# Iheckzza/FeatureMatching

Hardware: AMD Instinct MI355X
Metric: image-pairs/sec at 640x480 (coarse corr + dual-softmax mutual-NN + fine window refinement) (higher is better)
Workload: dtype i8 screening + f32 exact; 1 GPU; 640x480 pair, C=256 @1/8 (L=S=4800), Cf=64 @1/2, 5x5 fine window, 'peaky' descriptors; launch=hipGraph replay, concurrent_streams=4, fine_maps_layout=nchw

## Files before the change

featurematching_amd/_lib.py:

```python
from __future__ import annotations

import ctypes as C
import os

_HERE = os.path.dirname(os.path.abspath(__file__))
LIB_PATH = os.path.join(_HERE, "lib", "libfmatch_hip.so")

FM_OK = 0
FM_F32, FM_F16, FM_BF16 = 0, 1, 2
FM_E_CAPACITY = -5
FM_E_CANDIDATES = -6
FM_E_RANGE = -7
FM_E_DENSE = -8
FM_E_INTERNAL = -9
FM_E_STEP = -10
FM_DEV_RANGE = 4
FM_DEV_ALL_DENSE = 256
FM_MODE_EXACT_SCREENING, FM_MODE_DENSE, FM_MODE_NO_CELL_MAPS, FM_MODE_EXACT_STEP, FM_MODE_STATS = 1, 2, 4, 8, 16
FM_MODE_FLAT = 32
FM_MODE_ALONE = 64
FM_LOSS_CROSS_ENTROPY, FM_LOSS_FOCAL = 0, 1
FM_LAYOUT_NCHW_PREPARED = 2

_lib = None
# ... 12 lines not shown
                             _p, C.c_size_t, _i, _i, _p, _p, _p, _p, _p, _p, _i, _p, _p, _p]),
    "fm_coarse_match_dtype": (_i, [_p, _p, _i, _i, _i, _i, _i, _i, _i, _i, _i, _f, _f, _i, _f, _p, _p,
                                   _p, C.c_size_t, _i, _i, _p, _p, _p, _p, _p, _p, _i, _p, _p, _p]),
    "fm_coarse_match_maps": (_i, [_p, _p, _i, _i, _i, _i, _i, _i, _i, _i, _i, _f, _f, _i, _f, _p, _p,
                                  _p, C.c_size_t, _i, _i, _p, _p, _p, _p, _p, _p, _i, _p, _p, _p, _i, _i, _i, _i, _p, _p]),
    "fm_coarse_workspace_bytes_auto": (_i, [_i, _i, _i, _i, _i, C.POINTER(C.c_size_t)]),
    "fm_coarse_match_auto": (_i, [_p, _p, _i, _i, _i, _i, _i, _i, _i, _i, _i, _f, _f, _i, _f, _p, _p,
                                  _p, C.c_size_t, _i, _i, _p, _p, _p, _p, _p, _p, _i, _p, _p,
                                  C.POINTER(C.c_int32), C.POINTER(C.c_int32), C.POINTER(C.c_int32), _p]),
    "fm_debug_coarse_layout": (_i, [_i, _i, _i, _i, _i, C.POINTER(C.c_int64), _i]),
    "fm_debug_launch_corr": (_i, [_p, _i, _i, _i, _i, _i, _f, _f, _i, _p]),
    "fm_debug_launch_screen": (_i, [_p, _p, _p, _i, _i, _i, _i, _i, _f, _f, _p]),
    "fm_debug_launch_prep": (_i, [_p, _p, _p, _i, _i, _i, _i, _i, _p]),
    "fm_debug_launch_prep_f16": (_i, [_p, _p, _p, _i, _i, _i, _i, _i, _i, _p]),
    "fm_debug_reset_counters": (_i, [_p, _i, _i, _i, _i, _i, _p]),
    "fm_read_count": (_i, [_p, _i, C.POINTER(C.c_int32), _p]),
    "fm_read_count_info": (_i, [_p, _i, C.POINTER(C.c_int32), C.POINTER(C.c_int32), _p]),
    "fm_debug_launch_flat": (_i, [_p, _p, _p, _i, _i, _i, _i, _i, _f, _f, _i, _p]),
    "fm_coarse_softmax_stats": (_i, [_p, _i, _i, _i, _i, _i, C.POINTER(_p), C.POINTER(_p), C.POINTER(_i), C.POINTER(_p),
                                     C.POINTER(_p), C.POINTER(_i)]),
    "fm_dual_softmax_conf_at": (_i, [_p, _p, _i, _i, _i, _i, _f, _p, _p, _i, _p, _p, _i, _p, _p, _p, _i, _p, _p]),
    "fm_dual_softmax_backward_workspace_bytes": (C.c_size_t, [_i, _i, _i, _i]),
    "fm_dual_softmax_backward": (_i, [_p, _p, _i, _i, _i, _i, _f, _p, _p, _i, _p, _p, _i, _p, _p, _p, _p, _i, _p, C.c_size_t, _p,
                                      _p, _p]),
    "fm_dual_softmax_backward_dense": (_i, [_p, _p, _i, _i, _i, _i, _f, _p, _p, _i, _p, _p, _i, _p, _p, C.c_size_t, _p, _p, _p]),
    "fm_coarse_loss_workspace_bytes": (C.c_size_t, [_i, _i, _i, _i, _i]),
    "fm_coarse_loss_forward": (_i, [_p, _p, _i, _i, _i, _i, _f, _p, _p, _i, _p, _p, _i, _i, _f, _f, _f, _f, _p, _p, _p, _i, _p,
                                    C.c_size_t, _p, _p]),
    "fm_coarse_loss_backward": (_i, [_p, _p, _i, _i, _i, _i, _f, _p, _p, _i, _p, _p, _i, _i, _f, _f, _f, _f, _p, _p, _p, _i, _p,
                                     C.c_size_t, _p, _p, _p, _p]),
# ... 73 lines not shown
```

featurematching_amd/csrc/api.hip:

```cpp
#include <math.h>
#include <stdlib.h>
#include <string.h>

#include "fm_debug.h"
#include "fm_internal.h"

namespace fm {

int choose_splits(int N, int panels, int tiles, int target) {
  const int wg = N * panels;
#ifdef FM_TUNE_ENV
  if (const char* e = getenv("FM_TARGET_WGS")) target = atoi(e) > 0 ? atoi(e) : 256;
#endif
  int s = target / (wg > 0 ? wg : 1);
  if (s < 1) s = 1;
  const int smax = tiles / 2 > 0 ? tiles / 2 : 1;
  if (s > smax) s = smax;
  if (s > 32) s = 32;
  return s;
}

static int choose_screen_chunks(int N, int Lp, int nunits, int* units_per_chunk, bool alone) {
  const long nrb = (long)N * (Lp / 32);
  const int cu = nrb * ((nunits + 63) / 64) >= 1024 ? 64 : (alone && nrb * ((nunits + 7) / 8) <= 8192 ? 8 : 32);
// ... 6 lines not shown

CoarseWs coarse_layout(int N, int L, int S, int C, int slots, bool alone) {
  CoarseWs w;
  memset(&w, 0, sizeof(w));
  C = padded_channels(C);
  w.N = N; w.L = L; w.S = S; w.C = C; w.slots = slots;
  w.Lp = round_up(L, kPanelRows);
  w.Sp = round_up(S, kTileCols);
  w.panels = w.Lp / kPanelRows;
  w.tiles = w.Sp / kTileCols;
  w.splits = choose_splits(N, w.panels, w.tiles);
  {
    int target = N * w.panels >= kMaxPassSlots ? 10 * kMaxPassSlots : (alone ? kMaxPassSlots : kMaxPassTarget);
    if (target == kMaxPassTarget && w.tiles / choose_splits(N, w.panels, w.tiles, kMaxPassTarget) >= 32) target = kMaxPassSlots;
    w.splits0 = choose_splits(N, w.panels, w.tiles, target);
  }
#ifdef FM_TUNE_ENV
  if (const char* e = getenv("FM_TARGET_WGS0")) w.splits0 = choose_splits(N, w.panels, w.tiles, atoi(e) > 0 ? atoi(e) : kMaxPassTarget);
#endif
  w.splits_s = choose_screen_chunks(N, w.Lp, w.Sp / 32, &w.units_s, alone);
  const size_t rows = (size_t)N * w.Lp, cols = (size_t)N * w.Sp;
  const size_t nblk = (rows * slots + 255) / 256;
  size_t o = 0;
  auto take = [&](size_t bytes) { size_t at = o; o = align256(o + bytes); return at; };
  auto since = [&](size_t at) { return Span{at, o - at}; };
  w.cand_count = take(rows * 4);
  w.ccand_count = take(cols * 4);
  w.cand_count_b = take(rows * 4);
  w.ccand_count_b = take(cols * 4);
  w.dense_cnt = take((size_t)N * 4);
// ... 12 lines not shown
  w.counters[1] = Span{w.scalars, sizeof(Scalars)};
  w.prep_zero = since(w.cand_count);
  w.q0 = take(rows * C); w.q1 = take(cols * C);
  w.sigimg = take((size_t)N * 2 * 4);
  w.imgstat = take((size_t)N * 8 * 4);
  w.l1_0 = take(rows * 4); w.l1_1 = take(cols * 4);
  w.bstat0 = take(rows / 32 * 16); w.bstat1 = take(cols / 32 * 16);
  w.emarg = take((size_t)N * 4);
  w.rowS = take(0); w.colS = take(0);
  w.nmr = take(rows * 4); w.nmc = take(cols * 4);
  w.umax = take(rows / 32 * (cols / N / 32) * 4);
  w.cand_j = take(rows * slots * 4); w.cand_x = take(rows * slots * 4);
  w.ccand_i = take(cols * slots * 4); w.ccand_x = take(cols * slots * 4);
  w.thr_r = take(rows * 4); w.thr_c = take(cols * 4);
  w.wmaxb = take(rows / 32 * 4); w.cmaxu = take(cols / 32 * 4);
  w.common_total = o;
  w.hi0 = take(rows * C * 2); w.lo0 = take(rows * C * 2);
  w.hi1 = take(cols * C * 2); w.lo1 = take(cols * C * 2);
  w.f16inv = take((size_t)N * 4);
  w.rowB = take(rows * w.splits * 4); w.colB = take(cols * w.panels * kColParts * 4);
  w.rsum = take(rows * 4); w.csum = take(cols * 4);
  w.nmr2 = take(rows * 4); w.nmc2 = take(cols * 4);
  w.cand_j_b = take(rows * slots * 4); w.cand_x_b = take(rows * slots * 4);
  w.ccand_i_b = take(cols * slots * 4); w.ccand_x_b = take(cols * slots * 4);
  w.total = o;
  return w;
}

}

// ... 144 lines not shown
  if (cap > 0 && (!b_ids || !i_ids || !j_ids || !mkpts0_c || !mkpts1_c || !mconf)) return FM_E_NULL;
  if (cap < 0 || L != h0c * w0c || S != h1c * w1c) return FM_E_SHAPE;
  if (const int bad = check_coarse_shape(N, L, S, C, cand_slots)) return bad;
  if (!(thr > 0.f) || !(thr < 1.f) || !(temperature > 0.f)) return FM_E_UNSUPPORTED;
  if (mode & ~kKnownModes) return FM_E_UNSUPPORTED;
  const CoarsePlan p = plan_coarse(mode, conf_matrix != nullptr, cand_slots);
  const CoarseWs w = coarse_layout(N, L, S, C, cand_slots, p.alone);
  if (workspace_bytes < p.workspace_bytes(w) || ((uintptr_t)workspace & 255)) return FM_E_WORKSPACE;
  char* base = (char*)workspace;
  hipStream_t st = (hipStream_t)stream;
  const float inv_ct = 1.0f / ((float)C * temperature);
  const float thr_list = fminf(thr, p.list_cap);
#define FM_TRY(call) do { const hipError_t e_ = (call); if (e_ != hipSuccess) return (int)e_; } while (0)
  if (!resume) {
    FM_TRY(launch_prep(feat0, feat1, in_dtype, C, w, base, p.exact_step, p.flat, st));
    FM_TRY(launch_max_i8(w, base, st));
    if (p.flat) FM_TRY(launch_stab(w, base, inv_ct, thr, p.allow_dead, st));
    else FM_TRY(launch_screen(feat0, feat1, in_dtype, C, w, base, inv_ct, thr, p.dense, p.allow_dead, st));
  } else {
    FM_TRY(clear_spans(base, w.reassign, st));
  }
  if (p.prep_f16) FM_TRY(launch_prep_f16(feat0, feat1, in_dtype, C, w, base, p.f16_force, st));
  if (p.dense) FM_TRY(launch_dense(w, base, inv_ct, thr_list, st));
  if (p.reduce) FM_TRY(launch_reduce(w, base, inv_ct, st));
  if (p.rescreen) FM_TRY(launch_dense(w, base, inv_ct, thr_list, st, nullptr, 1));
  if (p.exact_lists) FM_TRY(launch_exact_lists(w, base, inv_ct, feat0, feat1, in_dtype, C, st));
  if (p.conf) {
    FM_TRY(launch_dense(w, base, inv_ct, thr, st, conf_matrix));
    FM_TRY(launch_conf_patch(w, base, inv_ct, conf_matrix, st));
  }
#undef FM_TRY
// ... 129 lines not shown
  CoarseWs w;
  if (const int bad = checked_layout(workspace && nm_r && sum_r && pitch_r && nm_c && sum_c && pitch_c, N, L, S, C,
                                     cand_slots, &w))
    return bad;
  *nm_r = (const float*)((char*)workspace + w.nmr); *sum_r = (const float*)((char*)workspace + w.rsum); *pitch_r = w.Lp;
  *nm_c = (const float*)((char*)workspace + w.nmc); *sum_c = (const float*)((char*)workspace + w.csum); *pitch_c = w.Sp;
  return FM_OK;
}

extern "C" int fm_debug_launch_corr(void* workspace, int N, int L, int S, int C, int cand_slots, float temperature,
                                    float thr, int mode, void* stream) {
  CoarseWs w;
  if (const int bad = checked_layout(workspace, N, L, S, C, cand_slots, &w)) return bad;
  if (mode < 0 || mode > 2) return FM_E_UNSUPPORTED;
  hipStream_t st = (hipStream_t)stream;
  if (mode == 0) return (int)launch_max_i8(w, (char*)workspace, st);
  if (mode == 1) return (int)launch_dense(w, (char*)workspace, 1.0f / ((float)C * temperature), thr, st);
  return (int)launch_dense(w, (char*)workspace, 1.0f / ((float)C * temperature), thr, st, nullptr, 1);
}

extern "C" int fm_debug_launch_screen(void* workspace, const float* feat0, const float* feat1, int N, int L, int S,
                                          int C, int cand_slots, float temperature, float thr, void* stream) {
  CoarseWs w;
  if (const int bad = checked_layout(workspace && feat0 && feat1, N, L, S, C, cand_slots, &w)) return bad;
  return (int)launch_screen(feat0, feat1, FM_F32, C, w, (char*)workspace, 1.0f / ((float)C * temperature), thr, 1, 1,
                                (hipStream_t)stream);
}

extern "C" int fm_debug_launch_prep(void* workspace, const float* feat0, const float* feat1, int N, int L, int S, int C,
                                    int cand_slots, void* stream) {
  CoarseWs w;
// ... 9 lines not shown
}

extern "C" int fm_debug_launch_flat(void* workspace, const float* feat0, const float* feat1, int N, int L, int S, int C,
                                    int cand_slots, float temperature, float thr, int which, void* stream) {
  CoarseWs w;
  if (const int bad = checked_layout(workspace && feat0 && feat1, N, L, S, C, cand_slots, &w)) return bad;
  if (which < 0 || which > 1) return FM_E_UNSUPPORTED;
  if (which == 0) return (int)launch_prep(feat0, feat1, FM_F32, C, w, (char*)workspace, 0, 1, (hipStream_t)stream);
  return (int)launch_stab(w, (char*)workspace, 1.0f / ((float)C * temperature), thr, 1, (hipStream_t)stream);
}

extern "C" int fm_debug_reset_counters(void* workspace, int N, int L, int S, int C, int cand_slots, void* stream) {
  CoarseWs w;
  if (const int bad = checked_layout(workspace, N, L, S, C, cand_slots, &w)) return bad;
  return (int)clear_spans((char*)workspace, w.counters, (hipStream_t)stream);
}

extern "C" int fm_read_count(const int32_t* d_count, int cap, int32_t* m_out, void* stream) {
  return fm_read_count_info(d_count, cap, m_out, nullptr, stream);
}

extern "C" int fm_read_count_info(const int32_t* d_count, int cap, int32_t* m_out, int32_t* info_out, void* stream) {
  if (!d_count || !m_out) return FM_E_NULL;
  int32_t h[2] = {0, 0};
  hipStream_t st = (hipStream_t)stream;
  hipError_t e = hipMemcpyAsync(h, d_count, sizeof(h), hipMemcpyDeviceToHost, st);
  if (e != hipSuccess) return (int)e;
  e = hipStreamSynchronize(st);
  if (e != hipSuccess) return (int)e;
  *m_out = h[0];
// ... 11 lines not shown
```

featurematching_amd/csrc/coarse_max_i8.hip:

```cpp
#include <type_traits>

#include "fm_device.h"

namespace fm {

typedef int v4i __attribute__((ext_vector_type(4)));
typedef int v16i __attribute__((ext_vector_type(16)));

struct MaxArgs {
  const signed char* q0; const signed char* q1;
  unsigned* rowmax_u; unsigned* colmax_u; float* umax;
  const float4* bstat0; const float4* bstat1; float* imgstat;
  float* diag;
  int L, S, Lp, Sp, panels, tiles, splits, tiles_per_split, pgroup;
};

__device__ __forceinline__ int xcd_remap_m(int bid, int n) {
  const int q = n >> 3, rem = n & 7, x = bid & 7, y = bid >> 3;
  return (x < rem ? x * (q + 1) : rem * (q + 1) + (x - rem) * q) + y;
}
__device__ __forceinline__ int half_max32_hi_i(int v) {
  asm volatile("s_nop 1\n\tv_max_i32_dpp %0, %0, %0 quad_perm:[1,0,3,2] row_mask:0xf bank_mask:0xf\n\t"
               "s_nop 1\n\tv_max_i32_dpp %0, %0, %0 quad_perm:[2,3,0,1] row_mask:0xf bank_mask:0xf\n\t"
               "s_nop 1\n\tv_max_i32_dpp %0, %0, %0 row_half_mirror row_mask:0xf bank_mask:0xf\n\t"
               "s_nop 1\n\tv_max_i32_dpp %0, %0, %0 row_mirror row_mask:0xf bank_mask:0xf\n\t"
               "s_nop 1\n\tv_max_i32_dpp %0, %0, %0 row_bcast:15 row_mask:0xa bank_mask:0xf"
// ... 4 lines not shown
__device__ __forceinline__ int vmax3_i(int x, int y, int z) {
  int d;
  asm volatile("v_max3_i32 %0, %1, %2, %3" : "=v"(d) : "v"(x), "v"(y), "v"(z));
  return d;
}
__device__ __forceinline__ int halves_max_i(int v) {
  int p = v, q = v;
  asm volatile("s_nop 1\n\tv_permlane32_swap_b32 %0, %1" : "+v"(p), "+v"(q));
  return max(p, q);
}

#ifndef FM_MAX_EPI
#define FM_MAX_EPI 3
#endif

template <int C>
__global__ __launch_bounds__(256, 2) void k_max_i8(MaxArgs a) {
  constexpr int KS8 = C / 32;
  constexpr int TILE_BYTES = kTileCols * C;
  constexpr int NBUF = 4;
  constexpr int PIECES = 2 * KS8;
  constexpr int PER_WAVE = PIECES / 4;
  constexpr int PF = KS8 < 4 ? KS8 : 4;
  extern __shared__ __attribute__((aligned(16))) char smem[];
  __shared__ unsigned s_colmax[3 * 64 + 8];

  const int tid = threadIdx.x;
  const int lane = tid & 63;
  const int wv = __builtin_amdgcn_readfirstlane(tid >> 6);
  const int r = lane & 31, h = lane >> 5;
#ifdef FM_DIAG_CLOCK
// ... 106 lines not shown

  auto pipe = [&](auto do_next, auto do_cur, int un, v16i& an0, v16i& an1, int uc, v16i& ac0, v16i& ac1, int ts = -1, int tsbuf = 0) {
    constexpr bool DN = decltype(do_next)::value, DC = decltype(do_cur)::value;
    if (dead) {
      if (DN && DC && ts >= 0) stage(ts, tsbuf);
      return;
    }
    const unsigned base = lds0 + (((un >> 1) - t0) % NBUF) * TILE_BYTES + (un & 1) * (KS8 * 1024) + lane * 16;
    constexpr int RING = PF + 1;
    v4i bq[RING];
    auto issue_ = [](auto ksc, v4i (&bq_)[RING], unsigned base_) {
      constexpr int ks = decltype(ksc)::value;
      asm volatile("ds_read_b128 %0, %1 offset:%2" : "=v"(bq_[ks % RING]) : "v"(base_), "n"(ks * 1024));
    };
#define issue(...) issue_(__VA_ARGS__, bq, base)
    auto mask_edge = [&](v16i& ac, bool row_edge, int row00) {
      const int ucol0 = uc * 32;
      if (row_edge || ucol0 + 32 > a.S) {
        const bool cok = ucol0 + r < a.S;
#pragma unroll
        for (int g = 0; g < 16; ++g)
          if (!cok || row00 + (g & 3) + 8 * (g >> 2) + 4 * h >= a.L) ac[g] = kQMasked;
      }
    };
    int ta[8], tb[8], c0 = 0, c1 = 0, um = 0;
    auto R = [&](int k) {
      if (!(FM_MAX_EPI & 1)) { if (k == 0) { vmax_i(rstat0[0], ac0[0]); vmax_i(rstat1[0], ac1[0]); } return; }
      if (k < 16) vmax_i(rstat0[k], ac0[k]); else vmax_i(rstat1[k - 16], ac1[k - 16]);
    };
    auto T = [&](const v16i& ac, int (&t)[8], int i) {
      if (!(FM_MAX_EPI & 2)) { if (i == 0) t[7] = ac[15]; return; }
      if (i < 5) t[i] = vmax3_i(ac[3 * i], ac[3 * i + 1], ac[3 * i + 2]);
      else if (i == 5) t[5] = vmax3_i(t[0], t[1], t[2]);
      else if (i == 6) t[6] = vmax3_i(t[3], t[4], ac[15]);
      else { t[7] = t[5]; vmax_i(t[7], t[6]); }
    };
    auto dpp = [&](auto step) {
      constexpr int st = decltype(step)::value;
      if (st == 0) asm volatile("s_nop 1\n\tv_max_i32_dpp %0, %0, %0 quad_perm:[1,0,3,2] row_mask:0xf bank_mask:0xf" : "+v"(um));
      else if (st == 1) asm volatile("s_nop 1\n\tv_max_i32_dpp %0, %0, %0 quad_perm:[2,3,0,1] row_mask:0xf bank_mask:0xf" : "+v"(um));
      else if (st == 2) asm volatile("s_nop 1\n\tv_max_i32_dpp %0, %0, %0 row_half_mirror row_mask:0xf bank_mask:0xf" : "+v"(um));
      else if (st == 3) asm volatile("s_nop 1\n\tv_max_i32_dpp %0, %0, %0 row_mirror row_mask:0xf bank_mask:0xf" : "+v"(um));
      else asm volatile("s_nop 1\n\tv_max_i32_dpp %0, %0, %0 row_bcast:15 row_mask:0xa bank_mask:0xf" : "+v"(um));
    };
    using I0 = std::integral_constant<int, 0>; using I1 = std::integral_constant<int, 1>;
    using I2 = std::integral_constant<int, 2>; using I3 = std::integral_constant<int, 3>;
    using I4 = std::integral_constant<int, 4>;
    auto group = [&](int s) {
      if (s == 0) { mask_edge(ac0, row_edge0, wrow0); mask_edge(ac1, row_edge1, wrow0 + 32); }
      R(2 * s); R(2 * s + 1);
      if (s < 8) T(ac0, ta, s);
      if (s >= 4 && s < 12) T(ac1, tb, s - 4);
      if (!(FM_MAX_EPI & 2)) { if (s == 15) { vmax_i(rstat0[1], ta[7]); vmax_i(rstat1[1], tb[7]); } return; }
      if (s == 8) c0 = halves_max_i(ta[7]);
      if (s == 12) c1 = halves_max_i(tb[7]);
      if (s == 13) {
        asm volatile("ds_max_u32 %0, %1" ::"v"(colmax_a + ((((uc >> 1) - t0) % 3) * 64 + (uc & 1) * 32 + r) * 4),
                     "v"(q_encode(max(c0, c1))) : "memory");
        um = h ? c1 : c0;
        asm volatile("s_nop 1" : "+v"(um));
        dpp(I0{});
      }
      if (s == 14) dpp(I1{});
// ... 64 lines not shown
                   t + NBUF - 1 < t1 ? t + NBUF - 1 : -1, (t - t0 + NBUF - 1) % NBUF); DG_ADD(dg_mfma) }
      { DG_T0 tile_barrier(min(t + NBUF - 1, t1 - 1) - (t + 1)); DG_ADD(dg_bar) }
      if (t > t0) fold_columns(t - 1);
      { DG_T0 pipe(T_{}, T_{}, 2 * t + 2, accA0, accA1, 2 * t + 1, accB0, accB1); DG_ADD(dg_epi) }
    }
    const int t = t1 - 1;
    { DG_T0 pipe(T_{}, T_{}, 2 * t + 1, accB0, accB1, 2 * t, accA0, accA1); DG_ADD(dg_mfma) }
    { DG_T0 tile_barrier(0); DG_ADD(dg_bar) }
    if (t > t0) fold_columns(t - 1);
    { DG_T0 pipe(F_{}, T_{}, 0, accA0, accA1, 2 * t + 1, accB0, accB1); DG_ADD(dg_epi) }
    asm volatile("s_waitcnt lgkmcnt(0)" ::: "memory");
    __builtin_amdgcn_s_barrier();
    fold_columns(t1 - 1);
  }
  if (stat_wg && tid < 6) a.imgstat[(long)b * 8 + tid] = __uint_as_float(s_colmax[192 + tid]);

#ifdef FM_DIAG_CLOCK
  const unsigned long long dg_tail0 = __builtin_amdgcn_s_memtime();
#endif
  if (!dead) {
    int V[32];
#pragma unroll
    for (int g = 0; g < 16; ++g) { V[g] = rstat0[g]; V[16 + g] = rstat1[g]; }
    asm volatile("s_nop 1" ::: "memory");
#pragma unroll
    for (int m = 0; m < 16; ++m) asm volatile("s_nop 1\n\tv_permlane16_swap_b32 %0, %1" : "+v"(V[2 * m]), "+v"(V[2 * m + 1]));
    int W[16];
#pragma unroll
    for (int m = 0; m < 16; ++m) W[m] = max(V[2 * m], V[2 * m + 1]);
    asm volatile("s_nop 1" ::: "memory");
// ... 28 lines not shown
    if (row < a.L && Q > kQMasked)
      __hip_atomic_fetch_max(a.rowmax_u + (long)b * a.Lp + row, q_encode(Q), __ATOMIC_RELAXED, __HIP_MEMORY_SCOPE_AGENT);
  }
#ifdef FM_DIAG_CLOCK
  if (lane < 8) {
    const float vals[8] = {(float)(__builtin_amdgcn_s_memtime() - dg0), (float)dg_pro, (float)dg_mfma, (float)dg_epi,
                           (float)dg_bar, (float)(__builtin_amdgcn_s_memrealtime() - dgr0), (float)(dgr0 & 0xffffff), (float)(__builtin_amdgcn_s_memtime() - dg_tail0)};
    float vv = 0.f;
#pragma unroll
    for (int q = 0; q < 8; ++q) vv = lane == q ? vals[q] : vv;
    a.diag[((long)blockIdx.x * 4 + wv) * 8 + lane] = vv;
  }
#endif
}

hipError_t launch_max_i8(const CoarseWs& w, char* base, hipStream_t st) {
  MaxArgs a;
  a.q0 = (const signed char*)(base + w.q0); a.q1 = (const signed char*)(base + w.q1);
  a.rowmax_u = (unsigned*)(base + w.rowmax_u); a.colmax_u = (unsigned*)(base + w.colmax_u);
  a.umax = (float*)(base + w.umax);
  a.bstat0 = (const float4*)(base + w.bstat0); a.bstat1 = (const float4*)(base + w.bstat1);
  a.imgstat = (float*)(base + w.imgstat);
  a.diag = (float*)(base + w.rowB);
  a.L = w.L; a.S = w.S; a.Lp = w.Lp; a.Sp = w.Sp; a.panels = w.panels; a.tiles = w.tiles;
  a.tiles_per_split = (w.tiles + w.splits0 - 1) / w.splits0;
  a.splits = (w.tiles + a.tiles_per_split - 1) / a.tiles_per_split;
  {
    const int blocks_all = w.N * a.splits * w.panels;
    const float share = fmaxf(1.f, (float)blocks_all / 8.f);
    int pgr = (int)lroundf(sqrtf(share * (float)(a.tiles_per_split * kTileCols) / (float)kPanelRows));
    a.pgroup = pgr < 1 ? 1 : (pgr > w.panels ? w.panels : pgr);
    if (a.splits == 1) a.pgroup = w.panels;
  }
  const int blocks = w.N * a.splits * w.panels;
  hipError_t e = hipSuccess;
#define FM_MAX_CASE(CC)                                                                        \
  case CC: {                                                                                   \
    static unsigned long long lds_set = 0;                                                     \
    e = ensure_dynamic_lds(&k_max_i8<CC>, 4 * kTileCols * CC, &lds_set);                       \
    if (e != hipSuccess) return e;                                                             \
    hipLaunchKernelGGL(k_max_i8<CC>, dim3(blocks), dim3(256), 4 * kTileCols * CC, st, a);      \
    break;                                                                                     \
  }
  switch (w.C) {
    FM_MAX_CASE(64)
    FM_MAX_CASE(128)
    FM_MAX_CASE(256)
    default: return hipErrorInvalidValue;
  }
#undef FM_MAX_CASE
  return hipGetLastError();
}

}
```

featurematching_amd/csrc/coarse_screen.hip:

```cpp
#include <stdlib.h>
#include <string.h>

#include "fm_device.h"

namespace fm {

typedef int v4i __attribute__((ext_vector_type(4)));
typedef int v16i __attribute__((ext_vector_type(16)));

constexpr int kMaxExact = 24;

struct ScreenArgs {
  const signed char* q0; const signed char* q1;
  const void* src0; const void* src1; int c_in, in_dtype;
  const unsigned* rowmax_u; const unsigned* colmax_u;
  const float* sigimg;
  const float* imgstat;
  const float* l1_0; const float* l1_1;
  const float4* bstat0; const float4* bstat1;
  const float* umax;
  float* nmr; float* nmc; float* emarg;
  int* dense_cnt; Scalars* scal;
  int* rcount; int* rlist_j; float* rlist_x;
  int* ccount; int* clist_i; float* clist_x;
// ... 6 lines not shown
  const int q = n >> 3, rem = n & 7, x = bid & 7, y = bid >> 3;
  return (x < rem ? x * (q + 1) : rem * (q + 1) + (x - rem) * q) + y;
}

template <int CTRL, int BANK>
__device__ __forceinline__ float dpp_mov_s(float old, float v) {
  return __builtin_bit_cast(float, __builtin_amdgcn_update_dpp(__builtin_bit_cast(int, old), __builtin_bit_cast(int, v),
                                                               CTRL, 0xf, BANK, false));
}
__device__ __forceinline__ float half_reduce32_max(float v) {
  v = fmaxf(v, dpp_mov_s<0xB1, 0xf>(v, v));
  v = fmaxf(v, dpp_mov_s<0x4E, 0xf>(v, v));
  { float t = dpp_mov_s<0x104, 0x5>(v, v); t = dpp_mov_s<0x114, 0xA>(t, v); v = fmaxf(v, t); }
  v = fmaxf(v, dpp_mov_s<0x128, 0xf>(v, v));
  { float p = v, q = v; asm volatile("s_nop 1\n\tv_permlane16_swap_b32 %0, %1" : "+v"(p), "+v"(q)); v = fmaxf(p, q); }
  return v;
}
__device__ __forceinline__ float row_sum16(float v) {
  v = v + dpp_mov_s<0xB1, 0xf>(v, v);
  v = v + dpp_mov_s<0x4E, 0xf>(v, v);
  v = v + dpp_mov_s<0x141, 0xf>(v, v);
  v = v + dpp_mov_s<0x140, 0xf>(v, v);
  return v;
}

__device__ __forceinline__ int sig_threshold(float nm, float emu, float inv_kss) {
  const float t = floorf((-kSkipLog2 - emu - nm) * inv_kss) - 1.f;
  return (int)fminf(fmaxf(t, -1.0e9f), 1.0e9f);
}

// ... 23 lines not shown
  if (idx < len) {
    const float ln2 = 0.69314718f;
    const float l1 = (side ? a.l1_1 : a.l1_0)[g];
    const unsigned mx = (side ? a.colmax_u : a.rowmax_u)[g];
    const bool dead = a.allow_dead && 2.002f * l1 * (side ? infA : infB) * a.inv_ct + 1e-3f <
                                          (a.lt + __builtin_log2f((float)(side ? a.L : a.S))) * ln2;
    const float mraw = side ? q8_margin_raw(sig0, l1A_max, clipA, sig1, l1, clipB, a.cpad)
                            : q8_margin_raw(sig0, l1, clipA, sig1, l1B_max, clipB, a.cpad);
    nm = dead ? -INFINITY : neg_stabiliser_log2(ss * q_decode(mx), mraw, a.inv_ct);
  }
  (side ? a.nmc : a.nmr)[g] = nm;
}

struct RowsExtra {
  int* thr_r; int* thr_c; float* wmaxb; float* cmaxu;
  int nchunks, chunk_units, items;
};

__global__ __launch_bounds__(256) void k_thresh(ScreenArgs a, RowsExtra x) {
  const int side = blockIdx.z, b = blockIdx.y;
  const int len = side ? a.S : a.L, lenp = side ? a.Sp : a.Lp;
  const int idx = blockIdx.x * 256 + threadIdx.x;
  const int lane = threadIdx.x & 63;
  const float sig0 = a.sigimg[b * 2], sig1 = a.sigimg[b * 2 + 1];
  const float* ist = a.imgstat + (long)b * 8;
  const float l1A_max = ist[0], clipA = ist[1], infA = ist[2], l1B_max = ist[3], clipB = ist[4], infB = ist[5];
  const float ss = sig0 * sig1;
  const float kss = a.k * ss;
  const bool screen_ok = kss > 1e-30f && kss < 1e30f;
  const float inv_kss = screen_ok ? 1.0f / kss : 0.f;
// ... 14 lines not shown
  float emu = 0.f;
  if (idx < len) {
    const float ln2 = 0.69314718f;
    const float l1 = (side ? a.l1_1 : a.l1_0)[g];
    const unsigned mx = (side ? a.colmax_u : a.rowmax_u)[g];
    const float bl1 = (side ? a.bstat1 : a.bstat0)[(long)b * nblk + blk].x;
    const bool dead = a.allow_dead && 2.002f * l1 * (side ? infA : infB) * a.inv_ct + 1e-3f <
                                          (a.lt + __builtin_log2f((float)(side ? a.L : a.S))) * ln2;
    const float mraw = side ? q8_margin_raw(sig0, l1A_max, clipA, sig1, l1, clipB, a.cpad)
                            : q8_margin_raw(sig0, l1, clipA, sig1, l1B_max, clipB, a.cpad);
    nm = dead ? -INFINITY : neg_stabiliser_log2(ss * q_decode(mx), mraw, a.inv_ct);
    emu = margin_log2(side ? q8_margin_raw(sig0, l1A_max, clipA, sig1, bl1, clipB, a.cpad)
                           : q8_margin_raw(sig0, bl1, clipA, sig1, l1B_max, clipB, a.cpad), a.inv_ct);
  }
  (side ? a.nmc : a.nmr)[g] = nm;
  (side ? x.thr_c : x.thr_r)[g] = idx < len ? sig_threshold(nm, emu, inv_kss) : 0x3fffffff;
  const float bm = half_reduce32_max(nm);
  if ((lane & 31) == 0) (side ? x.cmaxu : x.wmaxb)[(long)b * nblk + blk] = bm;
}

template <int C>
__global__ __launch_bounds__(256, 3) void k_screen_rows(ScreenArgs a, RowsExtra x) {
  constexpr int KS8 = C / 32;
  constexpr int LIST = 256;
  const int tid = threadIdx.x;
  const int lane = tid & 63;
  const int wv = __builtin_amdgcn_readfirstlane(tid >> 6);
  const int r = lane & 31, h = lane >> 5;
  __shared__ int s_list[4][LIST];

  const int nrb = a.Lp / 32, nunits = a.Sp / 32;
  const int item = xcd_remap_s(blockIdx.x, gridDim.x) * 4 + wv;
  if (item >= x.items) return;
// ... 4 lines not shown
  const int rb = kk - chunk * nrb;
  const int wrow0 = rb * 32;
  if (wrow0 >= a.L) return;
  const int u0 = chunk * x.chunk_units;
  const int U = min(x.chunk_units, nunits - u0);

  const float sig0 = a.sigimg[b * 2], sig1 = a.sigimg[b * 2 + 1];
  const float* ist = a.imgstat + (long)b * 8;
  const float clipA = ist[1], clipB = ist[4];
  const float bl1A = a.bstat0[(long)b * nrb + rb].x;
  const float wmax = x.wmaxb[(long)b * nrb + rb];
  const int ul_c = min(lane, U - 1);
  const float um = a.umax[((long)b * nrb + rb) * nunits + u0 + ul_c];
  const float cm = x.cmaxu[(long)b * nunits + u0 + ul_c];
  const float bl1B = a.bstat1[(long)b * nunits + u0 + ul_c].x;
  int trr[16];
  {
    const int* tp = x.thr_r + (long)b * a.Lp + wrow0 + 4 * h;
#pragma unroll
    for (int q = 0; q < 4; ++q) {
      const int4 t4 = *reinterpret_cast<const int4*>(tp + 8 * q);
      trr[4 * q] = t4.x; trr[4 * q + 1] = t4.y; trr[4 * q + 2] = t4.z; trr[4 * q + 3] = t4.w;
    }
  }
  v4i aq[KS8];
  {
    const signed char* src = a.q0 + (((long)b * a.Lp + wrow0) / 32 * KS8 * 64 + lane) * 16;
#pragma unroll
    for (int ks = 0; ks < KS8; ++ks) aq[ks] = *reinterpret_cast<const v4i*>(src + ks * 1024);
  }
  const float ss = sig0 * sig1;
  const float kss = a.k * ss;
  const bool screen_ok = kss > 1e-30f && kss < 1e30f;

  unsigned long long live;
  {
    const float emu = margin_log2(q8_margin_raw(sig0, bl1A, clipA, sig1, bl1B, clipB, a.cpad), a.inv_ct);
    const float top = __builtin_fmaf(um, kss, emu);
    const bool hot = lane < U && (!screen_ok || !((top + wmax < -kSkipLog2) && (top + cm < -kSkipLog2)));
    live = __ballot(hot);
  }
  const bool flat = !screen_ok || a.dense_cnt[b] != 0;
  int nd_units = flat ? 1 : 0;
  int nlist = 0;
#ifdef FM_ABL_ROWS
  if (FM_ABL_ROWS & 1) live = 0;
#endif
  if (!flat && live) {
    const bool row_edge = (wrow0 + 32 > a.L);
    const signed char* q1b = a.q1 + ((long)b * nunits + u0) * KS8 * 1024 + lane * 16;
    const int* tcb = x.thr_c + (long)b * a.Sp + u0 * 32 + r;
    auto load_unit = [&](int ul, v4i (&bq)[KS8], int& tcl) {
      const signed char* src = q1b + (long)ul * KS8 * 1024;
#pragma unroll
      for (int ks = 0; ks < KS8; ++ks) bq[ks] = *reinterpret_cast<const v4i*>(src + ks * 1024);
      tcl = tcb[ul * 32];
    };
    auto screen_unit = [&](int ul, const v4i (&bq)[KS8], int tcl) {
      const int ucol0 = (u0 + ul) * 32;
      v16i acc;
#pragma unroll
      for (int g = 0; g < 16; ++g) acc[g] = 0;
// ... 31 lines not shown
    int tcA = 0, tcB = 0;
    unsigned long long mask = live;
    int ulA = __builtin_ctzll(mask), ulB = -1;
    mask &= mask - 1;
    load_unit(ulA, bA, tcA);
    while (true) {
      ulB = -1;
      if (mask) { ulB = __builtin_ctzll(mask); mask &= mask - 1; load_unit(ulB, bB, tcB); }
      screen_unit(ulA, bA, tcA);
      if (ulB < 0 || nd_units) break;
      ulA = -1;
      if (mask) { ulA = __builtin_ctzll(mask); mask &= mask - 1; load_unit(ulA, bA, tcA); }
      screen_unit(ulB, bB, tcB);
      if (ulA < 0 || nd_units) break;
    }
    if (nd_units) nlist = 0;
  }

  int overflow = 0;
#ifdef FM_ABL_ROWS
  if (FM_ABL_ROWS & 2) nlist = 0;
#endif
  {
    constexpr int NPASS = 4;
    const int sub = lane >> 4, l16 = lane & 15;
    const int vpr = a.c_in >> 2;
    for (int e0 = 0; e0 < nlist; e0 += 4 * NPASS) {
      int myres = 0;
      float my_nmr = 0.f, my_nmc = 0.f;
      if (lane < 4 * NPASS && e0 + lane < nlist) {
        const int ky = s_list[wv][e0 + lane];
        const int row = wrow0 + ((ky >> 5) & 31), col = (u0 + ((ky >> 10) & 63)) * 32 + (ky & 31);
// ... 98 lines not shown

hipError_t launch_screen(const void* feat0, const void* feat1, int in_dtype, int c_in, const CoarseWs& w, char* base,
                         float inv_ct, float thr, int dense_enabled, int allow_dead, hipStream_t st) {
  ScreenArgs a;
  memset(&a, 0, sizeof(a));
  fill_screen_stats(a, w, base, inv_ct, thr, allow_dead);
  a.in_dtype = in_dtype;
  a.q0 = (const signed char*)(base + w.q0); a.q1 = (const signed char*)(base + w.q1);
  a.src0 = feat0; a.src1 = feat1; a.c_in = c_in;
  a.rcount = (int*)(base + w.cand_count); a.rlist_j = (int*)(base + w.cand_j); a.rlist_x = (float*)(base + w.cand_x);
  a.ccount = (int*)(base + w.ccand_count); a.clist_i = (int*)(base + w.ccand_i); a.clist_x = (float*)(base + w.ccand_x);
  a.dense_enabled = dense_enabled;
  RowsExtra x;
  x.thr_r = (int*)(base + w.thr_r); x.thr_c = (int*)(base + w.thr_c);
  x.wmaxb = (float*)(base + w.wmaxb); x.cmaxu = (float*)(base + w.cmaxu);
  x.chunk_units = w.units_s;
  x.nchunks = w.splits_s;
#ifdef FM_TUNE_ENV
  if (const char* ev = getenv("FM_ROWS_CHUNK")) { x.chunk_units = atoi(ev); x.nchunks = (w.Sp / 32 + x.chunk_units - 1) / x.chunk_units; }
#endif
  x.items = (int)((long)w.N * (w.Lp / 32) * x.nchunks);
  const int lenp = w.Lp > w.Sp ? w.Lp : w.Sp;
  hipLaunchKernelGGL(k_thresh, dim3((lenp + 255) / 256, w.N, 2), dim3(256), 0, st, a, x);
  const int blocks_r = (x.items + 3) / 4;
  switch (w.C) {
    case 64: hipLaunchKernelGGL(k_screen_rows<64>, dim3(blocks_r), dim3(256), 0, st, a, x); break;
    case 128: hipLaunchKernelGGL(k_screen_rows<128>, dim3(blocks_r), dim3(256), 0, st, a, x); break;
    case 256: hipLaunchKernelGGL(k_screen_rows<256>, dim3(blocks_r), dim3(256), 0, st, a, x); break;
    default: return hipErrorInvalidValue;
  }
// ... 5 lines not shown
```

featurematching_amd/csrc/fm_debug.h:

```cpp
#ifndef FM_DEBUG_H_
#define FM_DEBUG_H_

#include "fmatch.h"

#ifdef __cplusplus
extern "C" {
#endif

int fm_debug_coarse_layout(int N, int L, int S, int C, int cand_slots, int64_t* out, int n_out);

int fm_debug_launch_corr(void* workspace, int N, int L, int S, int C, int cand_slots,
                         float temperature, float thr, int mode, void* stream);
int fm_debug_launch_screen(void* workspace, const float* feat0, const float* feat1, int N, int L, int S,
                               int C, int cand_slots, float temperature, float thr, void* stream);
int fm_debug_launch_prep(void* workspace, const float* feat0, const float* feat1, int N, int L, int S, int C,
                         int cand_slots, void* stream);
int fm_debug_launch_prep_f16(void* workspace, const float* feat0, const float* feat1, int N, int L, int S, int C,
                             int cand_slots, int force, void* stream);
int fm_debug_reset_counters(void* workspace, int N, int L, int S, int C, int cand_slots, void* stream);
int fm_debug_launch_flat(void* workspace, const float* feat0, const float* feat1, int N, int L, int S, int C,
                         int cand_slots, float temperature, float thr, int which, void* stream);

#ifdef __cplusplus
}
#endif
#endif
```

featurematching_amd/csrc/fm_internal.h:

```cpp
#pragma once
#include <hip/hip_runtime.h>
#include <stddef.h>
#include <stdint.h>

#include <type_traits>

#include "fmatch.h"

namespace fm {

constexpr int kPanelRows = 256;
constexpr int kColParts = 1;
constexpr int kTieCap = 1023;
constexpr int kTileCols = 64;
constexpr float kLog2e = 1.4426950408889634f;
constexpr float kSkipLog2 = 32.f;
constexpr unsigned FM_INT_SCREEN_OVERFLOW = 16u;
constexpr unsigned FM_INT_LOOKBACK_TIMEOUT = 64u;
constexpr int kPrepSampleRows = 32;
constexpr float kPrepHeadroom = 1.5f;

inline int round_up(int x, int m) { return (x + m - 1) / m * m; }
inline int padded_channels(int c) { return c <= 64 ? 64 : (c <= 128 ? 128 : 256); }
inline bool valid_channels(int c) { return c >= 4 && c <= 256 && c % 4 == 0; }
// ... 8 lines not shown
inline bool with_window(int W, F&& f) {
  if (W == 5) f(int_c<5>{});
  else if (W == 7) f(int_c<7>{});
  else return false;
  return true;
}

inline bool crop_shape_ok(int N, int Hf, int Wf, int stride, int m_max) {
  return N > 0 && Hf > 0 && Wf > 0 && stride > 0 && m_max >= 0;
}

struct CoarseWs {
  int N, L, S, C, Lp, Sp, panels, tiles, splits, slots;
  int splits0;
  int splits_s, units_s;
  Span prep_zero;
  Span reassign[3];
  Span counters[2];
  size_t cand_count, ccand_count, cand_count_b, ccand_count_b, dense_cnt, scalars;
  size_t cell0, cell1;
  size_t ties0, ties1;
  size_t rowmax_u, colmax_u;
  size_t blocktot;
  size_t q0, q1;
  size_t sigimg;
  size_t imgstat;
  size_t l1_0, l1_1;
  size_t bstat0, bstat1;
  size_t emarg;
  size_t rowS, colS;
  size_t nmr, nmc;
  size_t umax;
  size_t cand_j, cand_x;
  size_t ccand_i, ccand_x;
  size_t thr_r, thr_c;
  size_t wmaxb, cmaxu;
  size_t common_total;
  size_t hi0, lo0, hi1, lo1;
  size_t f16inv;
  size_t rowB, colB;
  size_t rsum, csum;
  size_t nmr2, nmc2;
  size_t cand_j_b, cand_x_b, ccand_i_b, ccand_x_b;
  size_t total;
};

int choose_splits(int N, int panels, int tiles, int target = 256);
CoarseWs coarse_layout(int N, int L, int S, int C, int slots, bool alone = false);

struct Scalars {
  unsigned flags;
  int dense_units;
  int reserved;
};

hipError_t launch_prep(const void* feat0, const void* feat1, int in_dtype, int c_in, const CoarseWs& w, char* base,
                       int exact_step, int planes, hipStream_t st);
hipError_t launch_stab(const CoarseWs& w, char* base, float inv_ct, float thr, int allow_dead, hipStream_t st);
hipError_t launch_prep_f16(const void* feat0, const void* feat1, int in_dtype, int c_in, const CoarseWs& w, char* base,
                           int force, hipStream_t st);
hipError_t launch_max_i8(const CoarseWs& w, char* base, hipStream_t st);
hipError_t launch_dense(const CoarseWs& w, char* base, float inv_ct, float thr, hipStream_t st, float* conf = nullptr,
                        int rescreen = 0);
hipError_t launch_reduce(const CoarseWs& w, char* base, float inv_ct, hipStream_t st);
struct MapCopyJob {
  const float* src; float* dst; int N, Hf, Wf;
};
struct SelectFlags { bool exact, dense, cell_maps, sums_ready; };
hipError_t launch_select(const CoarseWs& w, char* base, int h0c, int w0c, int h1c, int w1c, float inv_ct, float thr, int border,
                         float scale_px, const float* scale0, const float* scale1,
                         int64_t* b_ids, int64_t* i_ids, int64_t* j_ids, float* k0, float* k1,
                         float* mconf, int cap, int32_t* d_count, SelectFlags flags, hipStream_t st,
                         const MapCopyJob* job = nullptr);
hipError_t launch_conf_patch(const CoarseWs& w, char* base, float inv_ct, float* conf, hipStream_t st);
hipError_t launch_exact_lists(const CoarseWs& w, char* base, float inv_ct, const void* feat0, const void* feat1, int in_dtype,
                              int c_in, hipStream_t st);
// ... 60 lines not shown
```

Measured before the change: 20340 image-pairs/s.

## Certify screen units via per-unit top-2 maxima to skip rescreening

The i8 max kernel gains a TOP2 variant that records, for each 32x32 unit, the largest and second-largest quantized score and the position of the largest. The screen kernel computes per-block minimum thresholds and marks a live unit as certified when its second max cannot pass that threshold. Certified units skip the full int8 rescreen and emit at most the single argmax candidate directly. This trades extra register and DPP reduction work in the max kernel, plus new workspace buffers, for fewer screen_unit passes on peaky descriptors.

```diff
diff --git a/featurematching_amd/_lib.py b/featurematching_amd/_lib.py
--- a/featurematching_amd/_lib.py
+++ b/featurematching_amd/_lib.py
@@ -50,6 +50,8 @@
     "fm_debug_launch_prep": (_i, [_p, _p, _p, _i, _i, _i, _i, _i, _p]),
     "fm_debug_launch_prep_f16": (_i, [_p, _p, _p, _i, _i, _i, _i, _i, _i, _p]),
     "fm_debug_reset_counters": (_i, [_p, _i, _i, _i, _i, _i, _p]),
+    "fm_debug_unit_cert": (_i, [_i]),
+    "fm_debug_unit_cert_layout": (_i, [_i, _i, _i, _i, _i, C.POINTER(C.c_int64), _i]),
     "fm_read_count": (_i, [_p, _i, C.POINTER(C.c_int32), _p]),
     "fm_read_count_info": (_i, [_p, _i, C.POINTER(C.c_int32), C.POINTER(C.c_int32), _p]),
     "fm_debug_launch_flat": (_i, [_p, _p, _p, _i, _i, _i, _i, _i, _f, _f, _i, _p]),
diff --git a/featurematching_amd/csrc/api.hip b/featurematching_amd/csrc/api.hip
--- a/featurematching_amd/csrc/api.hip
+++ b/featurematching_amd/csrc/api.hip
@@ -6,6 +6,8 @@
 #include "fm_internal.h"
 
 namespace fm {
+
+int g_unit_cert = 0;
 
 int choose_splits(int N, int panels, int tiles, int target) {
   const int wg = N * panels;
@@ -44,6 +46,7 @@
     int target = N * w.panels >= kMaxPassSlots ? 10 * kMaxPassSlots : (alone ? kMaxPassSlots : kMaxPassTarget);
     if (target == kMaxPassTarget && w.tiles / choose_splits(N, w.panels, w.tiles, kMaxPassTarget) >= 32) target = kMaxPassSlots;
     w.splits0 = choose_splits(N, w.panels, w.tiles, target);
+    w.top2 = N * w.panels < kMaxPassSlots && w.tiles / choose_splits(N, w.panels, w.tiles, kMaxPassTarget) < 32;
   }
 #ifdef FM_TUNE_ENV
   if (const char* e = getenv("FM_TARGET_WGS0")) w.splits0 = choose_splits(N, w.panels, w.tiles, atoi(e) > 0 ? atoi(e) : kMaxPassTarget);
@@ -86,6 +89,9 @@
   w.ccand_i = take(cols * slots * 4); w.ccand_x = take(cols * slots * 4);
   w.thr_r = take(rows * 4); w.thr_c = take(cols * 4);
   w.wmaxb = take(rows / 32 * 4); w.cmaxu = take(cols / 32 * 4);
+  w.tmin_r = take(rows / 32 * 4); w.tmin_c = take(cols / 32 * 4);
+  w.umax2 = take(rows / 32 * (cols / N / 32) * 4);
+  w.upos = take(rows / 32 * (cols / N / 32) * 4);
   w.common_total = o;
   w.hi0 = take(rows * C * 2); w.lo0 = take(rows * C * 2);
   w.hi1 = take(cols * C * 2); w.lo1 = take(cols * C * 2);
@@ -260,7 +266,7 @@
 #define FM_TRY(call) do { const hipError_t e_ = (call); if (e_ != hipSuccess) return (int)e_; } while (0)
   if (!resume) {
     FM_TRY(launch_prep(feat0, feat1, in_dtype, C, w, base, p.exact_step, p.flat, st));
-    FM_TRY(launch_max_i8(w, base, st));
+    FM_TRY(launch_max_i8(w, base, unit_cert_on(w, !p.dense), st));
     if (p.flat) FM_TRY(launch_stab(w, base, inv_ct, thr, p.allow_dead, st));
     else FM_TRY(launch_screen(feat0, feat1, in_dtype, C, w, base, inv_ct, thr, p.dense, p.allow_dead, st));
   } else {
@@ -420,7 +426,7 @@
   if (const int bad = checked_layout(workspace, N, L, S, C, cand_slots, &w)) return bad;
   if (mode < 0 || mode > 2) return FM_E_UNSUPPORTED;
   hipStream_t st = (hipStream_t)stream;
-  if (mode == 0) return (int)launch_max_i8(w, (char*)workspace, st);
+  if (mode == 0) return (int)launch_max_i8(w, (char*)workspace, unit_cert_on(w), st);
   if (mode == 1) return (int)launch_dense(w, (char*)workspace, 1.0f / ((float)C * temperature), thr, st);
   return (int)launch_dense(w, (char*)workspace, 1.0f / ((float)C * temperature), thr, st, nullptr, 1);
 }
@@ -460,6 +466,23 @@
   CoarseWs w;
   if (const int bad = checked_layout(workspace, N, L, S, C, cand_slots, &w)) return bad;
   return (int)clear_spans((char*)workspace, w.counters, (hipStream_t)stream);
+}
+
+extern "C" int fm_debug_unit_cert(int mode) {
+  const int prev = g_unit_cert;
+  if (mode >= 0 && mode <= 2) g_unit_cert = mode;
+  return prev;
+}
+
+extern "C" int fm_debug_unit_cert_layout(int N, int L, int S, int C, int cand_slots, int64_t* out, int n_out) {
+  if (!out) return FM_E_NULL;
+  if (n_out < 9) return FM_E_SHAPE;
+  CoarseWs w;
+  if (const int bad = checked_layout(true, N, L, S, C, cand_slots, &w)) return bad;
+  const int64_t v[9] = {(int64_t)w.umax, (int64_t)w.umax2, (int64_t)w.upos, (int64_t)w.thr_r, (int64_t)w.thr_c,
+                        (int64_t)w.tmin_r, (int64_t)w.tmin_c, (int64_t)(w.scalars + offsetof(Scalars, cert_units)), w.top2};
+  for (int i = 0; i < 9; ++i) out[i] = v[i];
+  return FM_OK;
 }
 
 extern "C" int fm_read_count(const int32_t* d_count, int cap, int32_t* m_out, void* stream) {
diff --git a/featurematching_amd/csrc/coarse_max_i8.hip b/featurematching_amd/csrc/coarse_max_i8.hip
--- a/featurematching_amd/csrc/coarse_max_i8.hip
+++ b/featurematching_amd/csrc/coarse_max_i8.hip
@@ -10,6 +10,7 @@
 struct MaxArgs {
   const signed char* q0; const signed char* q1;
   unsigned* rowmax_u; unsigned* colmax_u; float* umax;
+  int* umax2; int* upos;
   const float4* bstat0; const float4* bstat1; float* imgstat;
   float* diag;
   int L, S, Lp, Sp, panels, tiles, splits, tiles_per_split, pgroup;
@@ -44,7 +45,7 @@
 #define FM_MAX_EPI 3
 #endif
 
-template <int C>
+template <int C, bool TOP2>
 __global__ __launch_bounds__(256, 2) void k_max_i8(MaxArgs a) {
   constexpr int KS8 = C / 32;
   constexpr int TILE_BYTES = kTileCols * C;
@@ -181,13 +182,14 @@
       asm volatile("ds_read_b128 %0, %1 offset:%2" : "=v"(bq_[ks % RING]) : "v"(base_), "n"(ks * 1024));
     };
 #define issue(...) issue_(__VA_ARGS__, bq, base)
+    constexpr int kMasked = TOP2 ? -(1 << 26) : kQMasked;
     auto mask_edge = [&](v16i& ac, bool row_edge, int row00) {
       const int ucol0 = uc * 32;
       if (row_edge || ucol0 + 32 > a.S) {
         const bool cok = ucol0 + r < a.S;
 #pragma unroll
         for (int g = 0; g < 16; ++g)
-          if (!cok || row00 + (g & 3) + 8 * (g >> 2) + 4 * h >= a.L) ac[g] = kQMasked;
+          if (!cok || row00 + (g & 3) + 8 * (g >> 2) + 4 * h >= a.L) ac[g] = kMasked;
       }
     };
     int ta[8], tb[8], c0 = 0, c1 = 0, um = 0;
@@ -213,7 +215,76 @@
     using I0 = std::integral_constant<int, 0>; using I1 = std::integral_constant<int, 1>;
     using I2 = std::integral_constant<int, 2>; using I3 = std::integral_constant<int, 3>;
     using I4 = std::integral_constant<int, 4>;
+    int m1a = 0, m2a = 0, m1b = 0, m2b = 0;
+    int n1a = 0, n2a = 0, n1b = 0, n2b = 0;
+    int um2 = 0;
+    auto E = [&](int e) {
+      if (e >= 32) return;
+      const int g = e & 15;
+      int& m1 = e < 16 ? m1a : m1b;
+      int& m2 = e < 16 ? m2a : m2b;
+      const int v = e < 16 ? ac0[g] : ac1[g];
+      if (g == 0) {
+        asm volatile("v_lshlrev_b32 %0, 4, %2\n\tv_mov_b32 %1, %3" : "=&v"(m1), "=&v"(m2) : "v"(v), "v"(kQMasked));
+      } else {
+        int key;
+        asm volatile("v_lshl_or_b32 %2, %3, 4, %4\n\tv_med3_i32 %1, %0, %1, %2\n\tv_max_i32 %0, %0, %2"
+                     : "+v"(m1), "+v"(m2), "=&v"(key) : "v"(v), "n"(g));
+      }
+    };
+    auto halves2 = [&](int m1, int m2, int& n1, int& n2) {
+      int p1 = m1, q1 = m1, p2 = m2, q2 = m2, t;
+      asm volatile("s_nop 1\n\tv_permlane32_swap_b32 %0, %1\n\tv_permlane32_swap_b32 %2, %3"
+                   : "+v"(p1), "+v"(q1), "+v"(p2), "+v"(q2));
+      asm volatile("v_min_i32 %0, %2, %3\n\tv_max_i32 %1, %2, %3" : "=&v"(t), "=&v"(n1) : "v"(p1), "v"(q1));
+      asm volatile("v_max3_i32 %0, %1, %2, %3" : "=v"(n2) : "v"(t), "v"(p2), "v"(q2));
+    };
+#define FM_TOP2_STEP(CTRL)                                                                                              \
+    { int t, b2;                                                                                                          \
+      asm volatile("s_nop 1\n\tv_min_i32_dpp %2, %0, %0 " CTRL "\n\tv_mov_b32_dpp %3, %1 " CTRL "\n\t"                     \
+                   "v_max_i32_dpp %0, %0, %0 " CTRL "\n\tv_max3_i32 %1, %2, %1, %3"                                       \
+                   : "+v"(um), "+v"(um2), "=&v"(t), "=&v"(b2)); }
+    auto dpp2 = [&](auto step) {
+      constexpr int st = decltype(step)::value;
+      if (st == 0) FM_TOP2_STEP("quad_perm:[1,0,3,2] row_mask:0xf bank_mask:0xf")
+      else if (st == 1) FM_TOP2_STEP("quad_perm:[2,3,0,1] row_mask:0xf bank_mask:0xf")
+      else if (st == 2) FM_TOP2_STEP("row_half_mirror row_mask:0xf bank_mask:0xf")
+      else if (st == 3) FM_TOP2_STEP("row_mirror row_mask:0xf bank_mask:0xf")
+      else FM_TOP2_STEP("row_bcast:15 row_mask:0xa bank_mask:0xf")
+    };
+#undef FM_TOP2_STEP
+    auto group2 = [&](int s) {
+      if (s == 0) { mask_edge(ac0, row_edge0, wrow0); mask_edge(ac1, row_edge1, wrow0 + 32); }
+      R(2 * s); R(2 * s + 1);
+      if (s < 11) { E(3 * s); E(3 * s + 1); E(3 * s + 2); }
+      if (s == 6) halves2(m1a, m2a, n1a, n2a);
+      if (s == 11) halves2(m1b, m2b, n1b, n2b);
+      if (s == 12) {
+        asm volatile("ds_max_u32 %0, %1" ::"v"(colmax_a + ((((uc >> 1) - t0) % 3) * 64 + (uc & 1) * 32 + r) * 4),
+                     "v"(q_encode(max(n1a, n1b) >> 4)) : "memory");
+        um = h ? n1b : n1a;
+        um2 = h ? n2b : n2a;
+        asm volatile("s_nop 1" : "+v"(um), "+v"(um2));
+        dpp2(I0{});
+      }
+      if (s == 13) { dpp2(I1{}); dpp2(I2{}); }
+      if (s == 14) { dpp2(I3{}); dpp2(I4{}); }
+      if (s == 15) {
+        asm volatile("s_nop 1" : "+v"(um));
+        const int k0 = __builtin_amdgcn_readlane(um, 31), k1 = __builtin_amdgcn_readlane(um, 63);
+        const unsigned long long w0 = __ballot(m1a == k0), w1 = __ballot(m1b == k1);
+        const int lw = h ? __builtin_ctzll(w1) : __builtin_ctzll(w0);
+        if (r == 31) {
+          const long at = ((long)b * (a.Lp / 32) + wrow0 / 32 + h) * nunits + uc;
+          const int v1 = um >> 4, v2 = um2 >> 4;
+          a.umax[at] = (float)(v1 <= kMasked ? kQMasked : v1);
+          a.umax2[at] = v2 <= kMasked ? kQMasked : v2;
+          a.upos[at] = (lw << 4) | (um & 15);
+        }
+      }
+    };
     auto group = [&](int s) {
+      if constexpr (TOP2) { group2(s); return; }
       if (s == 0) { mask_edge(ac0, row_edge0, wrow0); mask_edge(ac1, row_edge1, wrow0 + 32); }
       R(2 * s); R(2 * s + 1);
       if (s < 8) T(ac0, ta, s);
@@ -308,6 +379,7 @@
     fold_columns(t1 - 1);
   }
   if (stat_wg && tid < 6) a.imgstat[(long)b * 8 + tid] = __uint_as_float(s_colmax[192 + tid]);
+  if (stat_wg && tid == 6) a.imgstat[(long)b * 8 + 6] = TOP2 ? 1.f : 0.f;
 
 #ifdef FM_DIAG_CLOCK
   const unsigned long long dg_tail0 = __builtin_amdgcn_s_memtime();
@@ -366,11 +438,12 @@
 #endif
 }
 
-hipError_t launch_max_i8(const CoarseWs& w, char* base, hipStream_t st) {
+hipError_t launch_max_i8(const CoarseWs& w, char* base, bool top2, hipStream_t st) {
   MaxArgs a;
   a.q0 = (const signed char*)(base + w.q0); a.q1 = (const signed char*)(base + w.q1);
   a.rowmax_u = (unsigned*)(base + w.rowmax_u); a.colmax_u = (unsigned*)(base + w.colmax_u);
   a.umax = (float*)(base + w.umax);
+  a.umax2 = (int*)(base + w.umax2); a.upos = (int*)(base + w.upos);
   a.bstat0 = (const float4*)(base + w.bstat0); a.bstat1 = (const float4*)(base + w.bstat1);
   a.imgstat = (float*)(base + w.imgstat);
   a.diag = (float*)(base + w.rowB);
@@ -388,10 +461,16 @@
   hipError_t e = hipSuccess;
 #define FM_MAX_CASE(CC)                                                                        \
   case CC: {                                                                                   \
-    static unsigned long long lds_set = 0;                                                     \
-    e = ensure_dynamic_lds(&k_max_i8<CC>, 4 * kTileCols * CC, &lds_set);                       \
-    if (e != hipSuccess) return e;                                                             \
-    hipLaunchKernelGGL(k_max_i8<CC>, dim3(blocks), dim3(256), 4 * kTileCols * CC, st, a);      \
+    static unsigned long long lds_set[2] = {0, 0};                                             \
+    if (top2) {                                                                                \
+      e = ensure_dynamic_lds(&k_max_i8<CC, true>, 4 * kTileCols * CC, &lds_set[1]);            \
+      if (e != hipSuccess) return e;                                                           \
+      hipLaunchKernelGGL((k_max_i8<CC, true>), dim3(blocks), dim3(256), 4 * kTileCols * CC, st, a);  \
+    } else {                                                                                   \
+      e = ensure_dynamic_lds(&k_max_i8<CC, false>, 4 * kTileCols * CC, &lds_set[0]);           \
+      if (e != hipSuccess) return e;                                                           \
+      hipLaunchKernelGGL((k_max_i8<CC, false>), dim3(blocks), dim3(256), 4 * kTileCols * CC, st, a); \
+    }                                                                                          \
     break;                                                                                     \
   }
   switch (w.C) {
diff --git a/featurematching_amd/csrc/coarse_screen.hip b/featurematching_amd/csrc/coarse_screen.hip
--- a/featurematching_amd/csrc/coarse_screen.hip
+++ b/featurematching_amd/csrc/coarse_screen.hip
@@ -1,5 +1,7 @@
 #include <stdlib.h>
 #include <string.h>
+
+#include <type_traits>
 
 #include "fm_device.h"
 
@@ -44,6 +46,19 @@
   { float t = dpp_mov_s<0x104, 0x5>(v, v); t = dpp_mov_s<0x114, 0xA>(t, v); v = fmaxf(v, t); }
   v = fmaxf(v, dpp_mov_s<0x128, 0xf>(v, v));
   { float p = v, q = v; asm volatile("s_nop 1\n\tv_permlane16_swap_b32 %0, %1" : "+v"(p), "+v"(q)); v = fmaxf(p, q); }
+  return v;
+}
+__device__ __forceinline__ int half_reduce32_min_i(int v) {
+  auto mv = [](auto ctrl, auto bank, int old, int x) {
+    return __builtin_amdgcn_update_dpp(old, x, decltype(ctrl)::value, 0xf, decltype(bank)::value, false);
+  };
+  using std::integral_constant;
+  v = min(v, mv(integral_constant<int, 0xB1>{}, integral_constant<int, 0xf>{}, v, v));
+  v = min(v, mv(integral_constant<int, 0x4E>{}, integral_constant<int, 0xf>{}, v, v));
+  { int t = mv(integral_constant<int, 0x104>{}, integral_constant<int, 0x5>{}, v, v);
+    t = mv(integral_constant<int, 0x114>{}, integral_constant<int, 0xA>{}, t, v); v = min(v, t); }
+  v = min(v, mv(integral_constant<int, 0x128>{}, integral_constant<int, 0xf>{}, v, v));
+  { int p = v, q = v; asm volatile("s_nop 1\n\tv_permlane16_swap_b32 %0, %1" : "+v"(p), "+v"(q)); v = min(p, q); }
   return v;
 }
 __device__ __forceinline__ float row_sum16(float v) {
@@ -97,6 +112,10 @@
 
 struct RowsExtra {
   int* thr_r; int* thr_c; float* wmaxb; float* cmaxu;
+  int* tmin_r; int* tmin_c;
+  const int* umax2; const int* upos;
+  int look;
+  int count_cert;
   int nchunks, chunk_units, items;
 };
 
@@ -141,9 +160,14 @@
                            : q8_margin_raw(sig0, bl1, clipA, sig1, l1B_max, clipB, a.cpad), a.inv_ct);
   }
   (side ? a.nmc : a.nmr)[g] = nm;
-  (side ? x.thr_c : x.thr_r)[g] = idx < len ? sig_threshold(nm, emu, inv_kss) : 0x3fffffff;
+  const int thr = idx < len ? sig_threshold(nm, emu, inv_kss) : 0x3fffffff;
+  (side ? x.thr_c : x.thr_r)[g] = thr;
   const float bm = half_reduce32_max(nm);
-  if ((lane & 31) == 0) (side ? x.cmaxu : x.wmaxb)[(long)b * nblk + blk] = bm;
+  const int tm = half_reduce32_min_i(thr);
+  if ((lane & 31) == 0) {
+    (side ? x.cmaxu : x.wmaxb)[(long)b * nblk + blk] = bm;
+    (side ? x.tmin_c : x.tmin_r)[(long)b * nblk + blk] = tm;
+  }
 }
 
 template <int C>
@@ -178,6 +202,10 @@
   const float um = a.umax[((long)b * nrb + rb) * nunits + u0 + ul_c];
   const float cm = x.cmaxu[(long)b * nunits + u0 + ul_c];
   const float bl1B = a.bstat1[(long)b * nunits + u0 + ul_c].x;
+  const bool look = x.look && ist[6] != 0.f;
+  const int um2 = x.umax2[((long)b * nrb + rb) * nunits + u0 + ul_c];
+  const int upos = x.upos[((long)b * nrb + rb) * nunits + u0 + ul_c];
+  const int tmin = min(x.tmin_r[(long)b * nrb + rb], x.tmin_c[(long)b * nunits + u0 + ul_c]);
   int trr[16];
   {
     const int* tp = x.thr_r + (long)b * a.Lp + wrow0 + 4 * h;
@@ -204,12 +232,22 @@
     const bool hot = lane < U && (!screen_ok || !((top + wmax < -kSkipLog2) && (top + cm < -kSkipLog2)));
     live = __ballot(hot);
   }
+  const unsigned long long cert = look ? (live & __ballot(um2 <= tmin)) : 0ull;
+  live &= ~cert;
   const bool flat = !screen_ok || a.dense_cnt[b] != 0;
   int nd_units = flat ? 1 : 0;
   int nlist = 0;
 #ifdef FM_ABL_ROWS
   if (FM_ABL_ROWS & 1) live = 0;
 #endif
+  int cert_thr = 0x3fffffff, cert_key = 0;
+  if (!flat && ((cert >> lane) & 1)) {
+    const int g = upos & 15, lw = (upos >> 4) & 63;
+    const int rl = (g & 3) + 8 * (g >> 2) + 4 * (lw >> 5), cl = lw & 31;
+    cert_thr = min(x.thr_r[(long)b * a.Lp + wrow0 + rl], x.thr_c[(long)b * a.Sp + (u0 + lane) * 32 + cl]);
+    cert_key = (lane << 10) | (rl << 5) | cl;
+  }
+  if (x.count_cert && cert && lane == 0) atomicAdd(&a.scal->cert_units, __builtin_popcountll(cert));
   if (!flat && live) {
     const bool row_edge = (wrow0 + 32 > a.L);
     const signed char* q1b = a.q1 + ((long)b * nunits + u0) * KS8 * 1024 + lane * 16;
@@ -271,8 +309,17 @@
       screen_unit(ulB, bB, tcB);
       if (ulA < 0 || nd_units) break;
     }
-    if (nd_units) nlist = 0;
-  }
+  }
+  if (!flat && cert && !nd_units) {
+    const unsigned long long hits = __ballot((int)um > cert_thr);
+    const int nh = __builtin_popcountll(hits);
+    if (nlist + nh > LIST) ++nd_units;
+    else {
+      if ((hits >> lane) & 1) s_list[wv][nlist + __builtin_popcountll(hits & ((1ull << lane) - 1ull))] = cert_key;
+      nlist += nh;
+    }
+  }
+  if (nd_units) nlist = 0;
 
   int overflow = 0;
 #ifdef FM_ABL_ROWS
@@ -401,6 +448,10 @@
   RowsExtra x;
   x.thr_r = (int*)(base + w.thr_r); x.thr_c = (int*)(base + w.thr_c);
   x.wmaxb = (float*)(base + w.wmaxb); x.cmaxu = (float*)(base + w.cmaxu);
+  x.tmin_r = (int*)(base + w.tmin_r); x.tmin_c = (int*)(base + w.tmin_c);
+  x.umax2 = (const int*)(base + w.umax2); x.upos = (const int*)(base + w.upos);
+  x.look = g_unit_cert != 1;
+  x.count_cert = g_unit_cert == 2;
   x.chunk_units = w.units_s;
   x.nchunks = w.splits_s;
 #ifdef FM_TUNE_ENV
diff --git a/featurematching_amd/csrc/fm_debug.h b/featurematching_amd/csrc/fm_debug.h
--- a/featurematching_amd/csrc/fm_debug.h
+++ b/featurematching_amd/csrc/fm_debug.h
@@ -20,6 +20,8 @@
 int fm_debug_reset_counters(void* workspace, int N, int L, int S, int C, int cand_slots, void* stream);
 int fm_debug_launch_flat(void* workspace, const float* feat0, const float* feat1, int N, int L, int S, int C,
                          int cand_slots, float temperature, float thr, int which, void* stream);
+int fm_debug_unit_cert(int mode);
+int fm_debug_unit_cert_layout(int N, int L, int S, int C, int cand_slots, int64_t* out, int n_out);
 
 #ifdef __cplusplus
 }
diff --git a/featurematching_amd/csrc/fm_internal.h b/featurematching_amd/csrc/fm_internal.h
--- a/featurematching_amd/csrc/fm_internal.h
+++ b/featurematching_amd/csrc/fm_internal.h
@@ -46,6 +46,7 @@
   int N, L, S, C, Lp, Sp, panels, tiles, splits, slots;
   int splits0;
   int splits_s, units_s;
+  int top2;
   Span prep_zero;
   Span reassign[3];
   Span counters[2];
@@ -67,6 +68,8 @@
   size_t ccand_i, ccand_x;
   size_t thr_r, thr_c;
   size_t wmaxb, cmaxu;
+  size_t tmin_r, tmin_c;
+  size_t umax2, upos;
   size_t common_total;
   size_t hi0, lo0, hi1, lo1;
   size_t f16inv;
@@ -83,15 +86,20 @@
 struct Scalars {
   unsigned flags;
   int dense_units;
-  int reserved;
+  int cert_units;
 };
+
+extern int g_unit_cert;
+inline bool unit_cert_on(const CoarseWs& w, bool common_path = true) {
+  return g_unit_cert == 2 || (g_unit_cert == 0 && w.top2 != 0 && common_path);
+}
 
 hipError_t launch_prep(const void* feat0, const void* feat1, int in_dtype, int c_in, const CoarseWs& w, char* base,
                        int exact_step, int planes, hipStream_t st);
 hipError_t launch_stab(const CoarseWs& w, char* base, float inv_ct, float thr, int allow_dead, hipStream_t st);
 hipError_t launch_prep_f16(const void* feat0, const void* feat1, int in_dtype, int c_in, const CoarseWs& w, char* base,
                            int force, hipStream_t st);
-hipError_t launch_max_i8(const CoarseWs& w, char* base, hipStream_t st);
+hipError_t launch_max_i8(const CoarseWs& w, char* base, bool top2, hipStream_t st);
 hipError_t launch_dense(const CoarseWs& w, char* base, float inv_ct, float thr, hipStream_t st, float* conf = nullptr,
                         int rescreen = 0);
 hipError_t launch_reduce(const CoarseWs& w, char* base, float inv_ct, hipStream_t st);
```

After: 20660 image-pairs/s, median of 6. 1.02x the previous value.
